# protolambda/go-kzg

Measured on AMD Instinct MI355X. Metric: KZG commitments/sec (CommitToPoly, 4096-element blob); FK20 half: value_fk20_4096, higher is better.
Workload: dtype u32; 1 GPU; CommitToPoly, 4096-coeff blobs, eth/trusted_setup.json monomial setup (s=1337), 4096 blobs/step/GPU resident in HBM, fixed-base table budget 110 GB (library default 110 GB: signed 16-bit windows, 8 of them walked by both GLV halves of every scalar, 103 GB; see table_sweep); global_batch=4096, parallelism=dp1 (independent blobs, no data-path collective)

## Files before the change

go-kzg_amd/__init__.py:

```python
import ctypes as C
import os

import numpy as np

_HERE = os.path.dirname(os.path.abspath(__file__))
LIB_PATH = os.environ.get("KZG_HIP_LIB") or os.path.join(_HERE, "libkzg_hip.so")

OK, ERR_TOO_WIDE, ERR_NOT_POW2, ERR_LEN_MISMATCH, ERR_UPPER_HALF, ERR_BAD_ARG, ERR_BAD_POINT, ERR_NO_DEVICE, ERR_HIP, ERR_UNSUPPORTED, ERR_RECOVERY, ERR_BAD_BLOB = range(12)


class KzgError(Exception):

    def __init__(self, status, msg=""):
        super().__init__("kzg_hip status %d %s" % (status, msg))
        self.status = status


class KzgPanic(KzgError):
    """The reference panics (kzg.go:22-27,44-52,74-91; fk20_single.go:60-62,140-154; bls_kilic.go:133-135)."""


class NoDeviceError(KzgError):
    pass

# ... 47 lines not shown
        "kzg_hip_check_proof_multi_interpolation": (i32, [vp, vp, u64, vp, vp, vp]),
        "kzg_hip_toeplitz_part2": (i32, [vp, vp, vp, u64, vp]), "kzg_hip_toeplitz_part3": (i32, [vp, vp, u64, vp]),
        "kzg_hip_fk20_single_settings_new": (i32, [vp, u64, pp]), "kzg_hip_fk20_single_settings_free": (None, [vp]),
        "kzg_hip_fk20_single_x_ext_fft": (i32, [vp, vp]), "kzg_hip_fk20_single": (i32, [vp, vp, u64, vp]),
        "kzg_hip_fk20_single_batch": (i32, [vp, vp, u64, u64, vp]), "kzg_hip_fk20_single_batch_dev": (i32, [vp, vp, u64, u64, vp, vp]),
        "kzg_hip_fk20_single_da_optimized": (i32, [vp, vp, u64, vp]), "kzg_hip_da_using_fk20": (i32, [vp, vp, u64, vp]),
        "kzg_hip_da_using_fk20_batch": (i32, [vp, vp, u64, u64, vp]), "kzg_hip_da_using_fk20_batch_dev": (i32, [vp, vp, u64, u64, vp, vp]),
        "kzg_hip_fk20_multi_settings_new": (i32, [vp, u64, u64, pp]), "kzg_hip_fk20_multi_settings_free": (None, [vp]),
        "kzg_hip_fk20_multi": (i32, [vp, vp, u64, vp]), "kzg_hip_fk20_multi_da_optimized": (i32, [vp, vp, u64, vp]),
        "kzg_hip_da_using_fk20_multi": (i32, [vp, vp, u64, vp]),
        "kzg_hip_da_using_fk20_multi_batch_dev": (i32, [vp, vp, u64, u64, vp, vp]),
        "kzg_hip_fk20_multi_hext_slice_dev": (i32, [vp, vp, u64, u64, u64, vp, vp]),
        "kzg_hip_fk20_multi_finish_dev": (i32, [vp, vp, i32, vp, vp]),
        "kzg_hip_eth_settings_new": (i32, [vp, vp, u64, pp]), "kzg_hip_eth_settings_free": (None, [vp]),
        "kzg_hip_eth_blob_to_kzg_commitment_batch": (i32, [vp, vp, u64, vp, vp]),
        "kzg_hip_eth_compute_kzg_proof": (i32, [vp, vp, u64, vp, vp, vp]),
        "kzg_hip_eth_compute_kzg_proof_batch": (i32, [vp, vp, u64, u64, vp, vp, vp, vp]),
        "kzg_hip_eth_compute_kzg_proof_batch_dev": (i32, [vp, vp, u64, u64, vp, vp, vp, vp, vp]),
        "kzg_hip_eth_compute_aggregate_kzg_proof": (i32, [vp, vp, u64, vp, vp]),
        "kzg_hip_eth_compute_aggregated_poly_and_commitment": (i32, [vp, vp, vp, u64, vp, vp, vp, vp]),
        "kzg_hip_test_sha256": (None, [vp, u64, vp]),
        "kzg_hip_evaluate_poly_in_evaluation_form": (i32, [vp, vp, u64, vp, u32, vp]),
        "kzg_hip_eth_evaluate_polynomial_in_evaluation_form": (i32, [vp, vp, u64, vp, vp]),
        "kzg_hip_bench_threads_fft_fr": (i32, [vp, vp, u64, u64, u32, u32, vp, C.POINTER(C.c_double)]),
        "kzg_hip_bench_drop_in_eth_proof": (i32, [vp, vp, u64, u64, u32, u32, vp, C.POINTER(C.c_double)]),
        "kzg_hip_zero_poly_via_multiplication": (i32, [vp, vp, u64, u64, vp, vp]),
        "kzg_hip_recover_poly_from_samples": (i32, [vp, vp, vp, u64, vp]),
        "kzg_hip_calibrate": (i32, [vp, C.POINTER(C.c_double), C.POINTER(C.c_double), C.POINTER(C.c_double)]),
        "kzg_hip_bench_drop_in": (i32, [vp, i32, vp, u64, u64, u32, u32, vp, C.POINTER(C.c_double)]),
        "kzg_hip_coalesce_stats": (i32, [vp, i32, C.POINTER(u64)]),
        "kzg_hip_lincomb_promotions": (i32, [vp, C.POINTER(u64), C.POINTER(u64)]),
        "kzg_hip_test_fp_inv": (i32, [vp, vp, u64, vp, vp, C.POINTER(C.c_double), C.POINTER(C.c_double)]),
        "kzg_hip_test_fr_inv": (i32, [vp, vp, u64, vp, vp, vp]),
        "kzg_hip_kzg_table_info": (i32, [vp, C.POINTER(C.c_uint32), C.POINTER(C.c_uint32), C.POINTER(u64)]), "kzg_hip_kzg_table_additions": (u32, [vp]), "kzg_hip_kzg_set_projective_outputs": (i32, [vp, i32]),
        "kzg_hip_da_using_fk20_multi_batch": (i32, [vp, vp, u64, u64, vp]),
        "kzg_hip_multi_settings_new": (i32, [C.POINTER(i32), u32, u32, vp, u64, pp]), "kzg_hip_multi_settings_free": (None, [vp]),
        "kzg_hip_multi_device_count": (u32, [vp]), "kzg_hip_multi_device": (i32, [vp, u32]),
        "kzg_hip_multi_fft": (vp, [vp, u32]), "kzg_hip_multi_kzg": (vp, [vp, u32]),
        "kzg_hip_multi_transport": (C.c_char_p, [vp]), "kzg_hip_multi_transport_note": (C.c_char_p, [vp]), "kzg_hip_multi_transport_check": (C.c_char_p, [vp]), "kzg_hip_multi_exchanges": (u64, [vp]),
        "kzg_hip_multi_set_fft_sharding": (i32, [vp, i32]), "kzg_hip_multi_set_table_budget_gb": (i32, [vp, C.c_double]),
        "kzg_hip_multi_commit_to_poly_batch": (i32, [vp, vp, u64, u64, vp]),
        "kzg_hip_multi_compute_proof_single_batch": (i32, [vp, vp, u64, u64, vp, vp]),
        "kzg_hip_multi_fft_fr_batch": (i32, [vp, vp, u64, u64, i32, vp]), "kzg_hip_multi_das_fft_extension_batch": (i32, [vp, vp, u64, u64]),
        "kzg_hip_multi_eth_settings_new": (i32, [vp, vp, u64, pp]), "kzg_hip_multi_eth_settings_free": (None, [vp]),
        "kzg_hip_multi_eth_blob_to_kzg_commitment_batch": (i32, [vp, vp, u64, vp, vp]),
        "kzg_hip_multi_eth_compute_kzg_proof_batch": (i32, [vp, vp, u64, u64, vp, vp, vp, vp]),
        "kzg_hip_multi_fk20_single_settings_new": (i32, [vp, u64, pp]), "kzg_hip_multi_fk20_single_settings_free": (None, [vp]),
        "kzg_hip_multi_da_using_fk20_batch": (i32, [vp, vp, u64, u64, vp]), "kzg_hip_multi_da_using_fk20": (i32, [vp, vp, u64, vp]),
        "kzg_hip_multi_fk20_multi_settings_new": (i32, [vp, u64, u64, pp]), "kzg_hip_multi_fk20_multi_settings_free": (None, [vp]),
        "kzg_hip_multi_da_using_fk20_multi_batch": (i32, [vp, vp, u64, u64, vp]), "kzg_hip_multi_da_using_fk20_multi": (i32, [vp, vp, u64, vp]),
        "kzg_hip_bench_poly_lincomb_dev": (i32, [vp, vp, u64, vp, u64, u64, vp, vp]),
        "kzg_hip_prof_reset": (None, [vp, i32]), "kzg_hip_prof_read": (i32, [vp, C.c_char_p, C.POINTER(C.c_double), C.POINTER(u64)]),
    }
    for name, (res, args) in sig.items():
        if os.environ.get("KZG_HIP_LIB_ALLOW_MISSING") and not hasattr(L, name):
            continue
        f = getattr(L, name)
        f.restype, f.argtypes = res, args
    _lib = L
    return L


API_SYMBOLS = None


def device_count():
# ... 707 lines not shown
```

go-kzg_amd/csrc/capi_bench.hip:

```cpp
#include "capi_common.hpp"

namespace {
struct prof_rec { std::string name; hipEvent_t e0, e1; };
std::mutex g_prof_mu;
bool g_prof_on = false;
std::vector<prof_rec> g_prof;
}
namespace kzg {
void prof_begin(hipStream_t s, const char *name) {
    if (!g_prof_on) return;
    std::lock_guard<std::mutex> lk(g_prof_mu);
    prof_rec r; r.name = name;
    hipEventCreate(&r.e0); hipEventCreate(&r.e1);
    hipEventRecord(r.e0, s);
    g_prof.push_back(r);
}
void prof_end(hipStream_t s, const char *name) {
    if (!g_prof_on) return;
    std::lock_guard<std::mutex> lk(g_prof_mu);
    for (size_t i = g_prof.size(); i-- > 0;)
        if (g_prof[i].name == name) { hipEventRecord(g_prof[i].e1, s); break; }
}
}

// ... 150 lines not shown
    HIPCHK(hipMemcpyAsync(d_in.p, in_fp, n * sizeof(fp), hipMemcpyHostToDevice, s));
    hipEvent_t e0, e1;
    HIPCHK(hipEventCreate(&e0)); HIPCHK(hipEventCreate(&e1));
    for (int which = 0; which < 2; which++) {
        void *out = which ? out_lane : out_coop; double *ms = which ? ms_lane : ms_coop;
        if (!out) continue;
        hipEventRecord(e0, s);
        launch_fp_inv_both(s, d_in.p, d_a.p, d_b.p, n, which ? 2 : 1);
        hipEventRecord(e1, s);
        HIPCHK(hipMemcpyAsync(out, which ? d_b.p : d_a.p, n * sizeof(fp), hipMemcpyDeviceToHost, s));
        HIPCHK(hipStreamSynchronize(s));
        float t = 0; hipEventElapsedTime(&t, e0, e1);
        if (ms) *ms = t;
    }
    hipEventDestroy(e0); hipEventDestroy(e1);
    HIPCHK(hipGetLastError());
    return KZG_HIP_OK;
}
int kzg_hip_test_fr_inv(kzg_hip_fft *fs, const void *in_fr, uint64_t n, void *out_coop, void *out_lane, void *out_block) {
    if (!fs || !in_fr || !n || n > (1u << 20) || !out_coop || !out_lane || !out_block) return KZG_HIP_ERR_BAD_ARG;
    dev_guard g(fs);
    hipStream_t s = fs->stream;
    dtmp<fr> d_in(s), d_a(s), d_b(s), d_c(s);
    CHK(d_in.alloc(n)); CHK(d_a.alloc(n)); CHK(d_b.alloc(n)); CHK(d_c.alloc(n));
    HIPCHK(hipMemcpyAsync(d_in.p, in_fr, n * sizeof(fr), hipMemcpyHostToDevice, s));
    launch_fr_inv_test(s, d_in.p, n, d_a.p, d_b.p, d_c.p);
    HIPCHK(hipGetLastError());
    HIPCHK(hipMemcpyAsync(out_coop, d_a.p, n * sizeof(fr), hipMemcpyDeviceToHost, s));
    HIPCHK(hipMemcpyAsync(out_lane, d_b.p, n * sizeof(fr), hipMemcpyDeviceToHost, s));
    HIPCHK(hipMemcpyAsync(out_block, d_c.p, n * sizeof(fr), hipMemcpyDeviceToHost, s));
    HIPCHK(hipStreamSynchronize(s));
    return KZG_HIP_OK;
}
int kzg_hip_coalesce_stats(kzg_hip_kzg *ks, int op, uint64_t out[8]) {
    if (!ks || !out || op < 0 || op > 1) return KZG_HIP_ERR_BAD_ARG;
    for (int i = 0; i < 8; i++) out[i] = 0;
    std::lock_guard<std::mutex> lk(ks->fs->mu);
    coalescer *co = op == 0 ? ks->co_commit.get() : ks->co_proof.get();
    if (co) co->stats(out);
    return KZG_HIP_OK;
}
void kzg_hip_prof_reset(kzg_hip_fft *fs, int enable) {
    (void)fs;
    std::lock_guard<std::mutex> lk(g_prof_mu);
    for (auto &r : g_prof) { hipEventDestroy(r.e0); hipEventDestroy(r.e1); }
    g_prof.clear();
    g_prof_on = enable != 0;
}
int kzg_hip_prof_read(kzg_hip_fft *fs, const char *kernel, double *total_ms, uint64_t *launches) {
    if (!fs || !kernel) return KZG_HIP_ERR_BAD_ARG;
    std::lock_guard<std::mutex> lk(g_prof_mu);
    double tot = 0; uint64_t cnt = 0;
    for (auto &r : g_prof) {
        if (r.name != kernel) continue;
        HIPCHK(hipEventSynchronize(r.e1));
        float ms = 0;
        HIPCHK(hipEventElapsedTime(&ms, r.e0, r.e1));
        tot += ms; cnt++;
    }
    if (total_ms) *total_ms = tot;
    if (launches) *launches = cnt;
    return KZG_HIP_OK;
}
```

go-kzg_amd/csrc/capi_kzg.hip:

```cpp
#include "capi_common.hpp"

int kzg_settings_build(kzg_hip_fft *fs, const void *points_g1, uint64_t n, kzg_hip_kzg **out) {
    dev_guard g(fs);
    hipStream_t s = fs->stream;
    std::unique_ptr<kzg_hip_kzg, void (*)(kzg_hip_kzg *)> own(new kzg_hip_kzg, kzg_hip_kzg_settings_free);
    kzg_hip_kzg *ks = own.get();
    ks->fs = fs; ks->n_setup = n;
    dtmp<g1j> d_raw(s);
    CHK(d_raw.alloc(n));
    HIPCHK(hipMalloc((void **)&ks->d_secret, n * sizeof(g1j)));
    HIPCHK(hipMalloc((void **)&ks->d_secret_a, n * sizeof(g1a)));
    HIPCHK(hipMemcpyAsync(d_raw.p, points_g1, n * sizeof(g1j), hipMemcpyHostToDevice, s));
    launch_g1_from_kilic(s, d_raw.p, n);
    launch_g1_normalize(s, d_raw.p, ks->d_secret, n);
    launch_g1_to_affine(s, ks->d_secret, ks->d_secret_a, n);
    HIPCHK(hipGetLastError());
    HIPCHK(hipStreamSynchronize(s));
    *out = own.release();
    return KZG_HIP_OK;
}
int kzg_hip_kzg_settings_new(kzg_hip_fft *fs, const void *secret_g1, uint64_t n_setup, kzg_hip_kzg **out) {
    if (!fs || !out || !secret_g1) return KZG_HIP_ERR_BAD_ARG;
    *out = nullptr;
    if (n_setup < fs->W) return KZG_HIP_ERR_LEN_MISMATCH;
// ... 35 lines not shown
}
int ensure_fixed_table(kzg_hip_kzg *ks, hipStream_t) {
    if (ks->d_fixed || ks->fixed_plan.c == 0xffffffffu) return KZG_HIP_OK;
    hipStream_t s = ks->fs->stream;
    double budget_gb = ks->budget_gb >= 0.0 ? ks->budget_gb : table_budget_gb("KZG_HIP_FB_BUDGET_GB", FB_DEFAULT_BUDGET_GB, 24.0);
    if (ks->n_setup < 64) { ks->fixed_plan.c = 0xffffffffu; return KZG_HIP_OK; }
    const bool glv = fb_glv_enabled();
    for (uint32_t c = 16; c >= 5; c--) {
        if (glv ? (c == 14) : (c == 15)) continue;
        const uint32_t nwin = glv ? fb_windows_glv(c) : fb_windows(c);
        double bytes = (double)nwin * (double)ks->n_setup * (double)(1u << (c - 1)) * sizeof(g1a);
        if (bytes > budget_gb * 1e9) continue;
        msm_plan p{};
        p.c = c; p.nwin = nwin; p.nb = 1u << (c - 1); p.ngroups = 1; p.fixed = 1; p.glv = glv ? 1 : 0; p.table_n = ks->n_setup;
        size_t entries = (size_t)p.nwin * ks->n_setup * p.nb;
        g1a *tab = nullptr;
        if (hipMalloc((void **)&tab, entries * sizeof(g1a)) != hipSuccess) { (void)hipGetLastError(); continue; }
        hipError_t e = launch_fb_build(s, ks->d_secret_a, ks->n_setup, p.c, p.nwin, tab);
        if (e == hipSuccess) e = hipStreamSynchronize(s);
        if (e != hipSuccess) { (void)hipGetLastError(); hipFree(tab); continue; }
        ks->d_fixed = tab; ks->fixed_plan = p;
        return KZG_HIP_OK;
    }
    ks->fixed_plan.c = 0xffffffffu;
    return KZG_HIP_OK;
}

int commit_rows(kzg_hip_kzg *ks, hipStream_t s, const fr *d_sc, uint64_t n, uint64_t batch, g1j *d_out, uint64_t sc_stride, bool to_kilic) {
    CHK(ensure_fixed_table(ks, s));
    bool fixed = ks->d_fixed != nullptr;
    if (!sc_stride) sc_stride = n;
    msm_plan p = fixed ? ks->fixed_plan : classic_plan(ks->n_setup);
    if (!fixed && !msm_index_range_ok(p, n)) return KZG_HIP_ERR_TOO_WIDE;
    size_t ws_main = fixed ? fb_partials_bytes(n, batch) : msm_workspace_bytes(p, n, batch);
    dtmp<uint8_t> d_ws(s);
    CHK(d_ws.alloc(ws_main));
    if (fixed) launch_fb_msm(s, ks->d_fixed, p.table_n, p.c, p.nwin, d_sc, sc_stride, n, batch, d_ws.p, d_out, to_kilic, p.glv != 0, to_kilic && ks->projective.load(std::memory_order_relaxed));
    else launch_msm(s, p, ks->d_secret_a, d_sc, sc_stride, n, batch, d_ws.p, d_out, to_kilic);
    HIPCHK(hipGetLastError());
    return KZG_HIP_OK;
}
int kzg_hip_kzg_set_table_budget_gb(kzg_hip_kzg *ks, double gb) {
    if (!ks || !(gb >= 0.0)) return KZG_HIP_ERR_BAD_ARG;
    std::unique_lock<std::shared_mutex> tl(ks->tab_mu);
    dev_guard g(ks->fs);
    if (ks->d_fixed) { HIPCHK(hipDeviceSynchronize()); HIPCHK(hipFree(ks->d_fixed)); ks->d_fixed = nullptr; }
    ks->fixed_plan = msm_plan{};
    ks->budget_gb = gb;
    return KZG_HIP_OK;
}

int kzg_hip_commit_to_poly_batch_dev(kzg_hip_kzg *ks, const void *d_coeffs_fr, uint64_t n, uint64_t batch, void *d_out_g1, void *stream) {
    if (!ks || !d_out_g1) return KZG_HIP_ERR_BAD_ARG;
    if (n > ks->n_setup) return KZG_HIP_ERR_LEN_MISMATCH;
    if (!batch) return KZG_HIP_OK;
    if (n == 0 || !d_coeffs_fr) return KZG_HIP_ERR_BAD_ARG;
    dev_guard g(ks->fs);
    return commit_rows(ks, (hipStream_t)stream, (const fr *)d_coeffs_fr, n, batch, (g1j *)d_out_g1);
}
namespace {
std::mutex g_reg_mu;
std::map<uintptr_t, size_t> g_registered;
}
const void *host_mapped_pointer(const void *host, size_t bytes) {
    hipPointerAttribute_t a;
    if (hipPointerGetAttributes(&a, host) != hipSuccess) { (void)hipGetLastError(); return nullptr; }
    if (a.type != hipMemoryTypeHost || !a.devicePointer) return nullptr;
// ... 359 lines not shown
```

go-kzg_amd/csrc/internal.hpp:

```cpp
#pragma once
#include <hip/hip_runtime.h>
#include <stdint.h>
#include "field.hpp"
#include "g1.hpp"

namespace kzg {

void launch_fr_fft(hipStream_t s, const fr *in, uint64_t in_stride, uint64_t n_in, fr *out, uint64_t n, uint64_t batch,
                   const fr *roots, uint64_t W, const fr *scale, const uint32_t *tw4096 = nullptr, const fr *roots_l = nullptr);
void launch_das_ext(hipStream_t s, fr *vals, uint64_t n, uint64_t batch, const fr *expanded, const fr *reversed, uint64_t W,
                    const fr *inv_n, const uint32_t *tw2048 = nullptr);
void launch_toeplitz_coeffs(hipStream_t s, const fr *poly, uint64_t poly_stride, uint64_t n, uint64_t l, uint64_t batch, fr *out,
                            const fr *scale);
void launch_quotient_linear(hipStream_t s, const fr *poly, uint64_t poly_stride, uint64_t n, uint64_t batch, const fr *x, fr *q, uint64_t q_stride);
void launch_fr_from_u64(hipStream_t s, const uint64_t *in, uint64_t in_stride, fr *out, uint64_t n);
void launch_fr_zero_tails(hipStream_t s, fr *rows, uint64_t n_max, uint64_t batch, const uint64_t *lens, uint64_t lens_stride);
void launch_fr_any_nonzero(hipStream_t s, const fr *vals, uint64_t n, uint32_t *flag);
void launch_fr_powers(hipStream_t s, const fr *base, uint64_t n, fr *out);

void launch_fr_from_le32(hipStream_t s, const uint8_t *in, fr *out, uint64_t per_blob, uint64_t batch, uint32_t *bad);
void launch_fr_to_le32(hipStream_t s, const fr *in, uint8_t *out, uint64_t n);
void launch_fr_bitrev_gather(hipStream_t s, const fr *in, fr *out, uint64_t n);
constexpr uint64_t ZERO_TREE_LEAF = 16;
void launch_zero_leaves(hipStream_t s, const fr *expanded, uint64_t stride, const uint64_t *missing, uint64_t n_missing, uint64_t leaves, fr *a);
// ... 26 lines not shown
void launch_g1_stage_coop_dif(hipStream_t s, int lanes, g1j *data, uint64_t n, uint64_t batch, uint64_t m, const fr *roots, const int8_t *wnaf, uint64_t W, uint64_t total);
void launch_g1_stage_coop_dit(hipStream_t s, int lanes, g1j *data, uint64_t n, uint64_t batch, uint64_t m, const fr *roots, const int8_t *wnaf, uint64_t W, uint64_t total);
void launch_g1_direct_coop(hipStream_t s, int lanes, uint32_t wgs, size_t pad_lds, const g1j *src, uint64_t src_stride, uint64_t src_valid, g1j *dst, uint32_t logn, uint32_t logR,
                           uint64_t Ns, const fr *roots, uint64_t W, const fr *sc, uint64_t total, uint32_t logT, uint32_t logU);
void launch_g1_fft_direct(hipStream_t s, const g1j *in, uint64_t in_stride, uint64_t n_valid, g1j *data, g1j *tmp, uint64_t n, uint64_t batch, const fr *roots,
                          uint64_t W, const fr *scale, uint32_t max_logr = 4, int lanes = 1, uint32_t bits_done = 0, uint64_t n_out = 0);
void launch_g1_normalize(hipStream_t s, const g1j *in, g1j *out, uint64_t n, bool to_kilic = false);
void launch_fr_inv_test(hipStream_t s, const fr *in, uint64_t n, fr *out_coop, fr *out_lane, fr *out_block);
void launch_fp_inv_both(hipStream_t s, const fp *in, fp *out_coop, fp *out_lane, uint64_t n, int mode);
void launch_g1_from_kilic(hipStream_t s, g1j *data, uint64_t n);
void launch_g1_to_affine(hipStream_t s, const g1j *in, g1a *out, uint64_t n);
void launch_g1_compress(hipStream_t s, const g1j *in, uint8_t *out48, uint64_t n);
void launch_g1_decompress(hipStream_t s, const uint8_t *in48, g1j *out, uint64_t n, uint32_t *bad_flag);
void launch_g1_fixed_base_powers(hipStream_t s, const fr *powers, uint64_t n, g1j *out);

uint64_t device_simd_lanes();
inline uint64_t device_simds() { return device_simd_lanes() / 64; }
struct msm_plan {
    uint32_t c;
    uint32_t nwin;
    uint32_t nb;
    uint32_t ngroups;
    uint32_t fixed;
    uint32_t glv;
    uint64_t table_n;
};
inline bool msm_index_range_ok(const msm_plan &p, uint64_t n) { return n < (1ull << 27) && 2 * p.table_n < (1ull << 30); }
size_t msm_workspace_bytes(const msm_plan &p, uint64_t n, uint64_t batch);
void launch_msm(hipStream_t s, const msm_plan &p, const g1a *table, const fr *scalars, uint64_t sc_stride, uint64_t n, uint64_t batch, void *workspace, g1j *out,
                bool to_kilic);
void launch_msm_window_table(hipStream_t s, const g1a *pts, uint64_t n, uint32_t c, uint32_t nwin, g1j *tmp, g1a *out);

size_t fb_partials_bytes(uint64_t n, uint64_t batch);
hipError_t launch_fb_build(hipStream_t s, const g1a *pts, uint64_t n, uint32_t c, uint32_t nwin, g1a *table);
void launch_fb_msm(hipStream_t s, const g1a *table, uint64_t table_n, uint32_t c, uint32_t nwin, const fr *scalars, uint64_t sc_stride, uint64_t n,
                   uint64_t batch, void *partials, g1j *out, bool to_kilic, bool glv = false, bool projective = false);

void launch_fb_mul_vec(hipStream_t s, const g1a *table, uint64_t table_n, uint32_t c, uint32_t nwin, const fr *scalars, uint64_t row, uint64_t j0,
                       uint64_t cnt, uint64_t batch, g1j *out, bool glv = false);
void launch_fb_mul_vec_dif2(hipStream_t s, const g1a *table, uint64_t table_n, uint32_t c, uint32_t nwin, const fr *scalars, const fr *roots, uint64_t W,
                            uint64_t batch, g1j *out, bool glv = false);
void launch_fb_mul_vec_files(hipStream_t s, const g1a *table, uint64_t table_n, uint32_t c, uint32_t nwin, const fr *scalars, uint64_t row, uint64_t j0,
                             uint64_t cnt, uint64_t batch, g1j *out, bool glv = false);
void launch_g1_sum_files(hipStream_t s, const g1j *tmp, uint64_t nfiles, uint64_t cnt, uint64_t batch, g1j *out);

void prof_begin(hipStream_t s, const char *name);
void prof_end(hipStream_t s, const char *name);

}
```

go-kzg_amd/csrc/k_msm.hip:

```cpp
#include "internal.hpp"
#include "g1_quad.hpp"
#include "coop_inv.hpp"
#include <atomic>
#include <cstring>

namespace kzg {

#define MSM_SORT_T 1024
#define MSM_ACC_BLOCK 128
#define MSM_NB 128

struct fb_partial { uint32_t w[52]; uint32_t inf; };
__device__ __forceinline__ void fb_partial_store(fb_partial &o, const g1x_acc &a) {
#pragma unroll
    for (int i = 0; i < 13; i++) { o.w[i] = a.v.x.l[i]; o.w[13 + i] = a.v.y.l[i]; o.w[26 + i] = a.v.zz.l[i]; o.w[39 + i] = a.v.zzz.l[i]; }
    o.inf = a.inf ? 1u : 0u;
}
__device__ __forceinline__ void fb_partial_load(const fb_partial &p, g1xq &v) {
#pragma unroll
    for (int i = 0; i < 13; i++) { v.x.l[i] = p.w[i]; v.y.l[i] = p.w[13 + i]; v.zz.l[i] = p.w[26 + i]; v.zzz.l[i] = p.w[39 + i]; }
}

template <uint32_t DELTA, bool ROW> __device__ __forceinline__ uint32_t lane_down(uint32_t v) {
    if constexpr (ROW && DELTA < 16) return (uint32_t)__builtin_amdgcn_update_dpp((int)v, (int)v, 0x100 + DELTA, 0xf, 0xf, false);
// ... 459 lines not shown
    hipLaunchKernelGGL(k_msm_sort, dim3((uint32_t)batch), dim3(MSM_SORT_T), sh, s, p.ngroups, p.table_n, scalars, sc_stride, n, ws, L.per_blob, L.entries_off,
                       L.offsets_off, K2);
    uint32_t S = 1;
    while (S < 16 && batch * L.K * S * 2 <= 2 * device_simd_lanes()) S *= 2;
    uint64_t total = batch * L.K * S;
    static const int seg_mode = [] { const char *e = getenv("KZG_HIP_MSM_SEG"); return e ? atoi(e) : -1; }();
    prof_begin(s, "msm_accumulate");
    const bool balanced = seg_mode == 1 || (seg_mode < 0 && batch * L.nseg >= 2 * device_simd_lanes());
    if (balanced) {
        const uint64_t tseg = batch * L.nseg, tb = batch * L.K;
        hipLaunchKernelGGL(k_msm_accumulate_seg, dim3((uint32_t)((tseg + MSM_ACC_BLOCK - 1) / MSM_ACC_BLOCK)), dim3(MSM_ACC_BLOCK), 0, s, table, ws, L.per_blob,
                           L.entries_off, L.offsets_off, L.buckets_off, L.segs_off, K2, L.nseg, tseg);
        hipLaunchKernelGGL(k_msm_merge_segs, dim3((uint32_t)((tb + MSM_ACC_BLOCK - 1) / MSM_ACC_BLOCK)), dim3(MSM_ACC_BLOCK), 0, s, ws, L.per_blob, L.offsets_off,
                           L.buckets_off, L.segs_off, K, tb);
    } else
        hipLaunchKernelGGL(k_msm_accumulate, dim3((uint32_t)((total + MSM_ACC_BLOCK - 1) / MSM_ACC_BLOCK)), dim3(MSM_ACC_BLOCK), 0, s, table, ws, L.per_blob,
                           L.entries_off, L.offsets_off, L.buckets_off, K, S, total);
    prof_end(s, "msm_accumulate");
    static const int reduce_mode = [] { const char *e = getenv("KZG_HIP_MSM_REDUCE"); return !e ? -1 : !strcmp(e, "chunks") ? 1 : !strcmp(e, "scan") ? 0 : -1; }();
    if (reduce_mode == 1 || (reduce_mode < 0 && balanced && batch * p.ngroups * 32 >= device_simd_lanes())) {
        const uint64_t tg = batch * p.ngroups;
        hipLaunchKernelGGL(k_msm_reduce_chunks, dim3((uint32_t)((tg + 3) / 4)), dim3(MSM_NB), 0, s, ws, L.per_blob, L.buckets_off, L.gsum_off, p.ngroups, tg);
    } else
        hipLaunchKernelGGL(k_msm_reduce, dim3((uint32_t)(batch * p.ngroups)), dim3(MSM_NB), 0, s, ws, L.per_blob, L.buckets_off, L.gsum_off, p.ngroups);
    hipLaunchKernelGGL(k_msm_combine, dim3((uint32_t)((batch + 63) / 64)), dim3(256), 0, s, ws, L.per_blob, L.gsum_off, p.ngroups, batch, out, to_kilic ? 1 : 0);
}

#ifndef FB_BLOCK
#define FB_BLOCK 128
#endif
#ifndef FB_FINISH_LANES_MAX
#define FB_FINISH_LANES_MAX 4
#endif
#ifndef FB_KEEP
#define FB_KEEP 16
#endif
#ifndef FB_ACC_WAVES
#define FB_ACC_WAVES 2
#endif

__global__ __launch_bounds__(FB_BLOCK, 2) void k_fb_build_pass1(const g1a *rows, uint64_t lanes, uint32_t D, uint32_t S, g1a *table, fp *ztmp) {
    uint64_t t = blockIdx.x * (uint64_t)blockDim.x + threadIdx.x;
    const uint32_t segs = D / S;
    if (t >= lanes * segs) return;
    const uint64_t row = t / segs; const uint32_t seg = (uint32_t)(t % segs);
    g1a b = rows[row];
    g1j cur = to_jac(b);
    uint32_t k = seg * S + 1;
    if (k > 1) {
        cur = g1_inf();
#pragma nounroll
        for (int bit = 31 - __builtin_clz(k); bit >= 0; bit--) {
            cur = g1_dbl(cur);
            if ((k >> bit) & 1u) cur = g1_madd(cur, b);
        }
    }
    g1a *dst = table + row * D + (uint64_t)seg * S; fp *zd = ztmp + row * D + (uint64_t)seg * S;
#pragma nounroll
    for (uint32_t d = 0; d < S; d++) {
        g1a xy; xy.x = cur.x; xy.y = cur.y;
        dst[d] = xy; zd[d] = cur.z;
        cur = g1_madd(cur, b);
    }
}
__global__ __launch_bounds__(FB_BLOCK, 2) void k_fb_build_pass2(uint64_t lanes, uint32_t D, uint32_t S, g1a *table, fp *ztmp, fp *ptmp) {
    uint64_t t = blockIdx.x * (uint64_t)blockDim.x + threadIdx.x;
    if (t >= lanes * (D / S)) return;
    g1a *dst = table + t * S; fp *zd = ztmp + t * S; fp *pd = ptmp + t * S;
    fp acc = one<FpP>();
// ... 143 lines not shown
            if (cmag) {
#else
        g1a qn = table[((uint64_t)w0 * table_n + i) * D + (mag ? mag - 1 : 0)];
#pragma nounroll
        for (uint32_t w = w0; w < w1; w++) {
            g1a q = qn;
            const uint32_t cmag = mag, cng = ng;
            if (w + 1 < w1) {
                raw = scalar_bits(k, (w + 1) * c, c) + carry;
                if (raw > D) { carry = 1; mag = (1u << c) - raw; ng = 1; } else { carry = 0; mag = raw; ng = 0; }
                qn = table[((uint64_t)(w + 1) * table_n + i) * D + (mag ? mag - 1 : 0)];
            }
            if (cmag) {
#endif
                if (cng) q.y = neg<FpP>(q.y);
                acc.add(q);
            }
        }
    }
#ifdef KZG_REDUCE_WAVE_COOP
    fb_block_reduce_coop(acc, buf, &lds, tid);
#else
    fb_block_reduce_quad(acc, buf, tid);
#endif
    if (tid == 0) fb_partial_store(partials[blockIdx.x], acc);
}
__device__ __forceinline__ uint32_t mag_bits(const uint32_t (&m)[4], uint32_t off, uint32_t c) {
    const uint32_t idx = off >> 5, sh = off & 31;
    if (idx >= 4) return 0;
    uint64_t v = m[idx];
    if (idx + 1 < 4) v |= (uint64_t)m[idx + 1] << 32;
    return (uint32_t)(v >> sh) & ((1u << c) - 1u);
}
template <bool SPLIT> __global__ __launch_bounds__(FB_ACC_BLOCK, FB_ACC_WAVES) void k_fb_accumulate_glv(const g1a *table, uint64_t table_n, uint32_t c, uint32_t nwin, uint32_t D, const fr *scalars,
                                                            uint64_t sc_stride, uint64_t n, uint32_t blocks_per_blob, uint32_t wsplit, fb_partial *partials) {
    __shared__ fb_partial buf[64];
#ifdef KZG_REDUCE_WAVE_COOP
    __shared__ coop_lds lds;
#endif
    const uint32_t tid = threadIdx.x;
    const uint64_t blob = blockIdx.x / blocks_per_blob; const uint32_t blk = blockIdx.x % blocks_per_blob;
    const uint64_t L = (uint64_t)blocks_per_blob * FB_ACC_BLOCK;
    const fr *sc = scalars + blob * sc_stride;
    g1x_acc acc; acc.init();
    const uint32_t wpg = SPLIT ? (nwin + wsplit - 1) / wsplit : nwin;
    const uint64_t nvh = SPLIT ? n * wsplit : n;
    bool in_phi = false;
    const bool keep_ok = !SPLIT && nvh % L == 0 && nvh / L <= FB_KEEP;
    uint32_t kept[FB_KEEP][5];
    uint32_t slot = 0;
    for (uint64_t v = (uint64_t)blk * FB_ACC_BLOCK + tid; v < 2 * nvh; v += L) {
        const bool phi = v < nvh;
        const uint64_t vh = phi ? v : v - nvh;
        const uint64_t i = SPLIT ? vh % n : vh;
        const uint32_t w0 = SPLIT ? (uint32_t)(vh / n) * wpg : 0u;
        const uint32_t w1 = SPLIT ? (w0 + wpg < nwin ? w0 + wpg : nwin) : nwin;
        if (SPLIT && w0 >= w1) continue;
        if (in_phi && !phi) { if (!acc.inf) acc.v.x = mulq(acc.v.x, unpackq(glv_beta())); in_phi = false; }
        uint32_t m[4], sgn;
        if (keep_ok && !phi) {
            const uint32_t at = slot < FB_KEEP ? slot : 0; slot++;
#pragma unroll
            for (int j = 0; j < 4; j++) m[j] = kept[at][j];
            sgn = kept[at][4];
            if (slot == (uint32_t)(nvh / L)) slot = 0;
        } else {
            const glv_halves h = glv_split_signed(from_mont<FrP>(sc[i]));
#pragma unroll
            for (int j = 0; j < 4; j++) m[j] = phi ? h.k2[j] : h.k1[j];
            sgn = phi ? h.neg2 : h.neg1;
            if (keep_ok) {
                const uint32_t at = slot < FB_KEEP ? slot : 0; slot++;
#pragma unroll
                for (int j = 0; j < 4; j++) kept[at][j] = h.k1[j];
                kept[at][4] = h.neg1;
                if (slot == (uint32_t)(nvh / L)) slot = 0;
            }
        }
        uint32_t raw, carry = 0, mag, ng;
        if (SPLIT) {
#pragma nounroll
            for (uint32_t w = 0; w < w0; w++) carry = (mag_bits(m, w * c, c) + carry > D) ? 1u : 0u;
        }
        raw = mag_bits(m, w0 * c, c) + carry;
        if (raw > D) { carry = 1; mag = (1u << c) - raw; ng = 1; } else { carry = 0; mag = raw; ng = 0; }
        g1a qn = table[((uint64_t)w0 * table_n + i) * D + (mag ? mag - 1 : 0)];
#pragma nounroll
        for (uint32_t w = w0; w < w1; w++) {
            g1a q = qn;
            const uint32_t cmag = mag, cng = ng;
            if (w + 1 < w1) {
                raw = mag_bits(m, (w + 1) * c, c) + carry;
                if (raw > D) { carry = 1; mag = (1u << c) - raw; ng = 1; } else { carry = 0; mag = raw; ng = 0; }
                qn = table[((uint64_t)(w + 1) * table_n + i) * D + (mag ? mag - 1 : 0)];
            }
            if (cmag) {
                if (cng ^ sgn) q.y = neg<FpP>(q.y);
                acc.add(q);
                in_phi = phi;
            }
        }
    }
    if (in_phi && !acc.inf) acc.v.x = mulq(acc.v.x, unpackq(glv_beta()));
#ifdef KZG_REDUCE_WAVE_COOP
    fb_block_reduce_coop(acc, buf, &lds, tid);
#else
    fb_block_reduce_quad(acc, buf, tid);
#endif
    if (tid == 0) fb_partial_store(partials[blockIdx.x], acc);
}
__global__ __launch_bounds__(256) void k_fb_finish(const fb_partial *partials, uint32_t blocks_per_blob, uint64_t batch, g1j *out, int to_kilic) {
    __shared__ fb_partial buf[64];
    const uint64_t b = blockIdx.x;
#ifdef KZG_REDUCE_WAVE_COOP
    __shared__ coop_lds lds;
    coop_ctx c; c.L = &lds; c.wave = threadIdx.x >> 6; c.col = threadIdx.x & 63u; c.set = 0;
    const uint32_t col = c.col;
    g1x_acc acc; acc.init();
    acc.v = g1xq_from_affine(g1a_inf());
    const uint32_t rounds = (blocks_per_blob + 63) / 64;
#pragma nounroll
    for (uint32_t r = 0; r < rounds; r++) {
        const uint32_t j = r * 64 + col;
        const bool have = j < blocks_per_blob;
        const fb_partial &pj = partials[b * blocks_per_blob + (have ? j : 0)];
        g1xq w; fb_partial_load(pj, w);
        coop_acc_add(acc, w, !have || pj.inf != 0, c);
    }
    const uint32_t live = blocks_per_blob < 64 ? blocks_per_blob : 64;
    uint32_t off = 1;
// ... 282 lines not shown
                            j0, cnt, row, total, out);
    prof_end(s, "fb_mul_vec");
}

uint64_t device_simd_lanes() {
    static std::atomic<uint64_t> lanes_of_device[64];
    int dev = 0;
    (void)hipGetDevice(&dev);
    std::atomic<uint64_t> &slot = lanes_of_device[dev >= 0 && dev < 64 ? dev : 0];
    uint64_t lanes = slot.load(std::memory_order_relaxed);
    if (!lanes) {
        int cus = 256;
        if (hipDeviceGetAttribute(&cus, hipDeviceAttributeMultiprocessorCount, dev) != hipSuccess) { (void)hipGetLastError(); cus = 256; }
        lanes = (uint64_t)(cus > 0 ? cus : 256) * 4 * 64;
        slot.store(lanes, std::memory_order_relaxed);
    }
    return lanes;
}
static uint32_t fb_blocks_per_blob(uint64_t n, uint64_t batch, uint32_t *wsplit = nullptr) {
    static const uint64_t forced_lanes = [] { const char *e = getenv("KZG_HIP_FB_LANES"); return e ? strtoull(e, nullptr, 10) : 0ull; }();
    uint64_t lanes = forced_lanes ? forced_lanes : 2 * device_simd_lanes();
    if (lanes < FB_ACC_BLOCK) lanes = FB_ACC_BLOCK;
    uint64_t target = lanes / FB_ACC_BLOCK;
    uint64_t bpb = target / (batch ? batch : 1);
    uint32_t split = 1;
    while (split < 8 && (batch ? batch : 1) * n * split * 2 <= lanes) split *= 2;
    if (wsplit) *wsplit = split;
    uint64_t maxb = (n * split + FB_ACC_BLOCK - 1) / FB_ACC_BLOCK;
    if (bpb > maxb) bpb = maxb;
    if (bpb < 1) bpb = 1;
    return (uint32_t)bpb;
}
size_t fb_partials_bytes(uint64_t n, uint64_t batch) { return (((size_t)std::max(fb_blocks_per_blob(n, batch), fb_blocks_per_blob(2 * n, batch)) * batch * sizeof(fb_partial)) + 15) / 16 * 16; }

void launch_fb_msm(hipStream_t s, const g1a *table, uint64_t table_n, uint32_t c, uint32_t nwin, const fr *scalars, uint64_t sc_stride, uint64_t n,
                   uint64_t batch, void *partials, g1j *out, bool to_kilic, bool glv, bool projective) {
    if (!batch) return;
    const int fin = (to_kilic ? 1 : 0) | (projective ? 2 : 0);
    uint32_t split = 1;
    uint32_t bpb = fb_blocks_per_blob(glv ? 2 * n : n, batch, &split);
    if (split > nwin) split = nwin;
    prof_begin(s, "fb_accumulate");
    if (glv) {
        if (split > 1) hipLaunchKernelGGL(k_fb_accumulate_glv<true>, dim3((uint32_t)(batch * bpb)), dim3(FB_ACC_BLOCK), 0, s, table, table_n, c, nwin, 1u << (c - 1), scalars, sc_stride, n,
                                          bpb, split, (fb_partial *)partials);
        else hipLaunchKernelGGL(k_fb_accumulate_glv<false>, dim3((uint32_t)(batch * bpb)), dim3(FB_ACC_BLOCK), 0, s, table, table_n, c, nwin, 1u << (c - 1), scalars, sc_stride, n, bpb,
                                1u, (fb_partial *)partials);
    } else if (split > 1) hipLaunchKernelGGL(k_fb_accumulate<true>, dim3((uint32_t)(batch * bpb)), dim3(FB_ACC_BLOCK), 0, s, table, table_n, c, nwin, 1u << (c - 1), scalars, sc_stride, n,
                                      bpb, split, (fb_partial *)partials);
    else hipLaunchKernelGGL(k_fb_accumulate<false>, dim3((uint32_t)(batch * bpb)), dim3(FB_ACC_BLOCK), 0, s, table, table_n, c, nwin, 1u << (c - 1), scalars, sc_stride, n, bpb,
                            1u, (fb_partial *)partials);
    prof_end(s, "fb_accumulate");
    if (bpb <= FB_FINISH_LANES_MAX) hipLaunchKernelGGL(k_fb_finish_lanes, dim3((uint32_t)((batch + 63) / 64)), dim3(64), 0, s, (const fb_partial *)partials, bpb, batch, out, fin);
    else hipLaunchKernelGGL(k_fb_finish, dim3((uint32_t)batch), dim3(256), 0, s, (const fb_partial *)partials, bpb, batch, out, fin);
}
hipError_t launch_fb_build(hipStream_t s, const g1a *pts, uint64_t n, uint32_t c, uint32_t nwin, g1a *table) {
    uint32_t D = 1u << (c - 1);
    g1j *rows_j = nullptr; g1a *rows = nullptr; fp *ztmp = nullptr, *ptmp = nullptr;
    uint64_t lanes_all = (uint64_t)nwin * n;
    hipError_t e;
    if ((e = hipMallocAsync((void **)&rows_j, lanes_all * sizeof(g1j), s)) != hipSuccess) return e;
    if ((e = hipMallocAsync((void **)&rows, lanes_all * sizeof(g1a), s)) != hipSuccess) { hipFreeAsync(rows_j, s); return e; }
    launch_msm_window_table(s, pts, n, c, nwin, rows_j, rows);
    uint64_t per_win = n * D * sizeof(fp);
    uint32_t slab = (uint32_t)((1ull << 30) / (per_win ? per_win : 1));
    if (slab < 1) slab = 1;
    if (slab > nwin) slab = nwin;
    if ((e = hipMallocAsync((void **)&ztmp, (uint64_t)slab * per_win, s)) != hipSuccess) { hipFreeAsync(rows_j, s); hipFreeAsync(rows, s); return e; }
    if ((e = hipMallocAsync((void **)&ptmp, (uint64_t)slab * per_win, s)) != hipSuccess) { hipFreeAsync(rows_j, s); hipFreeAsync(rows, s); hipFreeAsync(ztmp, s); return e; }
    for (uint32_t w0 = 0; w0 < nwin; w0 += slab) {
        uint32_t ws = (w0 + slab <= nwin) ? slab : nwin - w0;
        uint64_t lanes = (uint64_t)ws * n;
        uint32_t S = D;
        while (S > 64 && lanes * (D / S) < (1ull << 20)) S >>= 1;
        dim3 g((uint32_t)((lanes * (D / S) + FB_BLOCK - 1) / FB_BLOCK)), b(FB_BLOCK);
        hipLaunchKernelGGL(k_fb_build_pass1, g, b, 0, s, rows + (uint64_t)w0 * n, lanes, D, S, table + (uint64_t)w0 * n * D, ztmp);
        hipLaunchKernelGGL(k_fb_build_pass2, g, b, 0, s, lanes, D, S, table + (uint64_t)w0 * n * D, ztmp, ptmp);
    }
    hipFreeAsync(rows_j, s); hipFreeAsync(rows, s); hipFreeAsync(ztmp, s); hipFreeAsync(ptmp, s);
    return hipGetLastError();
}

__global__ __launch_bounds__(MSM_ACC_BLOCK, 2) void k_msm_window_rows(const g1a *pts, uint64_t n, uint32_t c, uint32_t nwin, g1j *tmp) {
    uint64_t i = blockIdx.x * (uint64_t)blockDim.x + threadIdx.x;
    if (i >= n) return;
// ... 16 lines not shown
```

go-kzg_amd/csrc/kzg_hip_internal.h:

```cpp
#ifndef KZG_HIP_INTERNAL_H
#define KZG_HIP_INTERNAL_H
#include "../../include/kzg_hip.h"
#ifdef __cplusplus
extern "C" {
#endif
#pragma GCC visibility push(default)

void kzg_hip_prof_reset(kzg_hip_fft *fs, int enable);
int kzg_hip_prof_read(kzg_hip_fft *fs, const char *kernel, double *total_ms, uint64_t *launches);
int kzg_hip_calibrate(kzg_hip_fft *fs, double *mad_per_s, double *add_per_s, double *fp_mul_per_s);
int kzg_hip_bench_drop_in(kzg_hip_kzg *ks, int op, const void *blobs_fr, uint64_t n, uint64_t nblobs, unsigned threads, unsigned calls, void *out_g1,
                          double *seconds);
int kzg_hip_bench_drop_in_eth_proof(kzg_hip_eth *eth, const void *polys_fr, uint64_t n, uint64_t npolys, unsigned threads, unsigned calls, void *out48,
                                    double *seconds);
int kzg_hip_bench_threads_fft_fr(kzg_hip_fft *fs, const void *vals_fr, uint64_t n, uint64_t nrows, unsigned threads, unsigned calls, void *out_fr, double *seconds);
int kzg_hip_bench_poly_lincomb_dev(kzg_hip_fft *fs, const void *d_vectors_fr, uint64_t stride, const void *d_scalars_fr, uint64_t count, uint64_t n, void *d_out_fr,
                                   void *stream);
int kzg_hip_coalesce_stats(kzg_hip_kzg *ks, int op, uint64_t out[8]);
int kzg_hip_test_fp_inv(kzg_hip_fft *fs, const void *in_fp, uint64_t n, void *out_coop, void *out_lane, double *ms_coop, double *ms_lane);
int kzg_hip_lincomb_promotions(kzg_hip_fft *fs, uint64_t *promoted, uint64_t *served);
int kzg_hip_test_fr_inv(kzg_hip_fft *fs, const void *in_fr, uint64_t n, void *out_coop, void *out_lane, void *out_block);
void kzg_hip_test_sha256(const void *data, uint64_t len, void *out32);


#pragma GCC visibility pop
#ifdef __cplusplus
}
#endif
#endif
```

Baseline: 102,000 commitments/s.

## Precompute signed GLV window digits in a separate kernel before fixed-base accumulation

Adds a k_fb_digits kernel that does the GLV split and signed-window recoding once per scalar and writes int16 digits to a workspace buffer. The accumulate kernel then reads those digits instead of redoing the split and carry chain in every thread, and the FB_KEEP register cache of kept halves is removed. This is meant to take scalar decomposition and recoding arithmetic out of the accumulate hot loop and cut register pressure there. The cost is an extra kernel launch, extra HBM traffic for the digit buffer (processed in chunks capped at 1 GB), and more workspace.

Result: no change. 102,500 commitments/s (median of 6 runs) (+0.5%).

```diff
diff --git a/go-kzg_amd/__init__.py b/go-kzg_amd/__init__.py
--- a/go-kzg_amd/__init__.py
+++ b/go-kzg_amd/__init__.py
@@ -103,6 +103,7 @@
         "kzg_hip_lincomb_promotions": (i32, [vp, C.POINTER(u64), C.POINTER(u64)]),
         "kzg_hip_test_fp_inv": (i32, [vp, vp, u64, vp, vp, C.POINTER(C.c_double), C.POINTER(C.c_double)]),
         "kzg_hip_test_fr_inv": (i32, [vp, vp, u64, vp, vp, vp]),
+        "kzg_hip_test_fb_digits": (i32, [vp, vp, u64, u32, vp]),
         "kzg_hip_kzg_table_info": (i32, [vp, C.POINTER(C.c_uint32), C.POINTER(C.c_uint32), C.POINTER(u64)]), "kzg_hip_kzg_table_additions": (u32, [vp]), "kzg_hip_kzg_set_projective_outputs": (i32, [vp, i32]),
         "kzg_hip_da_using_fk20_multi_batch": (i32, [vp, vp, u64, u64, vp]),
         "kzg_hip_multi_settings_new": (i32, [C.POINTER(i32), u32, u32, vp, u64, pp]), "kzg_hip_multi_settings_free": (None, [vp]),
diff --git a/go-kzg_amd/csrc/capi_bench.hip b/go-kzg_amd/csrc/capi_bench.hip
--- a/go-kzg_amd/csrc/capi_bench.hip
+++ b/go-kzg_amd/csrc/capi_bench.hip
@@ -206,6 +206,20 @@
     HIPCHK(hipStreamSynchronize(s));
     return KZG_HIP_OK;
 }
+int kzg_hip_test_fb_digits(kzg_hip_fft *fs, const void *scalars_fr, uint64_t n, uint32_t c, void *out_i16) {
+    if (!fs || !scalars_fr || !n || n > (1u << 20) || c < 2 || c > 16 || !out_i16) return KZG_HIP_ERR_BAD_ARG;
+    dev_guard g(fs);
+    hipStream_t s = fs->stream;
+    const uint32_t nwin = fb_windows_glv(c);
+    dtmp<fr> d_in(s); dtmp<int16_t> d_out(s);
+    CHK(d_in.alloc(n)); CHK(d_out.alloc(2ull * nwin * n));
+    HIPCHK(hipMemcpyAsync(d_in.p, scalars_fr, n * sizeof(fr), hipMemcpyHostToDevice, s));
+    launch_fb_digits(s, d_in.p, n, n, 1, c, nwin, d_out.p);
+    HIPCHK(hipGetLastError());
+    HIPCHK(hipMemcpyAsync(out_i16, d_out.p, 2ull * nwin * n * sizeof(int16_t), hipMemcpyDeviceToHost, s));
+    HIPCHK(hipStreamSynchronize(s));
+    return KZG_HIP_OK;
+}
 int kzg_hip_coalesce_stats(kzg_hip_kzg *ks, int op, uint64_t out[8]) {
     if (!ks || !out || op < 0 || op > 1) return KZG_HIP_ERR_BAD_ARG;
     for (int i = 0; i < 8; i++) out[i] = 0;
diff --git a/go-kzg_amd/csrc/capi_kzg.hip b/go-kzg_amd/csrc/capi_kzg.hip
--- a/go-kzg_amd/csrc/capi_kzg.hip
+++ b/go-kzg_amd/csrc/capi_kzg.hip
@@ -91,7 +91,7 @@
     if (!sc_stride) sc_stride = n;
     msm_plan p = fixed ? ks->fixed_plan : classic_plan(ks->n_setup);
     if (!fixed && !msm_index_range_ok(p, n)) return KZG_HIP_ERR_TOO_WIDE;
-    size_t ws_main = fixed ? fb_partials_bytes(n, batch) : msm_workspace_bytes(p, n, batch);
+    size_t ws_main = fixed ? fb_msm_workspace_bytes(n, batch, p.nwin, p.glv != 0) : msm_workspace_bytes(p, n, batch);
     dtmp<uint8_t> d_ws(s);
     CHK(d_ws.alloc(ws_main));
     if (fixed) launch_fb_msm(s, ks->d_fixed, p.table_n, p.c, p.nwin, d_sc, sc_stride, n, batch, d_ws.p, d_out, to_kilic, p.glv != 0, to_kilic && ks->projective.load(std::memory_order_relaxed));
diff --git a/go-kzg_amd/csrc/internal.hpp b/go-kzg_amd/csrc/internal.hpp
--- a/go-kzg_amd/csrc/internal.hpp
+++ b/go-kzg_amd/csrc/internal.hpp
@@ -82,9 +82,11 @@
 void launch_msm_window_table(hipStream_t s, const g1a *pts, uint64_t n, uint32_t c, uint32_t nwin, g1j *tmp, g1a *out);
 
 size_t fb_partials_bytes(uint64_t n, uint64_t batch);
+size_t fb_msm_workspace_bytes(uint64_t n, uint64_t batch, uint32_t nwin, bool glv);
+void launch_fb_digits(hipStream_t s, const fr *scalars, uint64_t sc_stride, uint64_t n, uint64_t batch, uint32_t c, uint32_t nwin, int16_t *digits);
 hipError_t launch_fb_build(hipStream_t s, const g1a *pts, uint64_t n, uint32_t c, uint32_t nwin, g1a *table);
 void launch_fb_msm(hipStream_t s, const g1a *table, uint64_t table_n, uint32_t c, uint32_t nwin, const fr *scalars, uint64_t sc_stride, uint64_t n,
-                   uint64_t batch, void *partials, g1j *out, bool to_kilic, bool glv = false, bool projective = false);
+                   uint64_t batch, void *workspace, g1j *out, bool to_kilic, bool glv = false, bool projective = false);
 
 void launch_fb_mul_vec(hipStream_t s, const g1a *table, uint64_t table_n, uint32_t c, uint32_t nwin, const fr *scalars, uint64_t row, uint64_t j0,
                        uint64_t cnt, uint64_t batch, g1j *out, bool glv = false);
diff --git a/go-kzg_amd/csrc/k_msm.hip b/go-kzg_amd/csrc/k_msm.hip
--- a/go-kzg_amd/csrc/k_msm.hip
+++ b/go-kzg_amd/csrc/k_msm.hip
@@ -515,9 +515,6 @@
 #ifndef FB_FINISH_LANES_MAX
 #define FB_FINISH_LANES_MAX 4
 #endif
-#ifndef FB_KEEP
-#define FB_KEEP 16
-#endif
 #ifndef FB_ACC_WAVES
 #define FB_ACC_WAVES 2
 #endif
@@ -727,8 +724,28 @@
     if (idx + 1 < 4) v |= (uint64_t)m[idx + 1] << 32;
     return (uint32_t)(v >> sh) & ((1u << c) - 1u);
 }
-template <bool SPLIT> __global__ __launch_bounds__(FB_ACC_BLOCK, FB_ACC_WAVES) void k_fb_accumulate_glv(const g1a *table, uint64_t table_n, uint32_t c, uint32_t nwin, uint32_t D, const fr *scalars,
-                                                            uint64_t sc_stride, uint64_t n, uint32_t blocks_per_blob, uint32_t wsplit, fb_partial *partials) {
+__device__ __forceinline__ void fb_recode_half(const uint32_t (&m)[4], uint32_t neg, uint32_t c, uint32_t nwin, int16_t *dst, uint64_t stride) {
+    const uint32_t D = 1u << (c - 1);
+    uint32_t carry = 0;
+#pragma nounroll
+    for (uint32_t w = 0; w < nwin; w++) {
+        const uint32_t raw = mag_bits(m, w * c, c) + carry;
+        carry = neg ? (raw > D ? 1u : 0u) : (raw >= D ? 1u : 0u);
+        const int32_t d = (int32_t)raw - (int32_t)(carry << c);
+        dst[(uint64_t)w * stride] = (int16_t)(neg ? -d : d);
+    }
+}
+__global__ __launch_bounds__(256) void k_fb_digits(const fr *scalars, uint64_t sc_stride, uint64_t n, uint64_t batch, uint32_t c, uint32_t nwin, int16_t *digits) {
+    const uint64_t t = (uint64_t)blockIdx.x * 256 + threadIdx.x;
+    if (t >= n * batch) return;
+    const uint64_t b = t / n, i = t - b * n;
+    const glv_halves h = glv_split_signed(from_mont<FrP>(scalars[b * sc_stride + i]));
+    int16_t *dst = digits + b * 2 * nwin * n + i;
+    fb_recode_half(h.k2, h.neg2, c, nwin, dst, n);
+    fb_recode_half(h.k1, h.neg1, c, nwin, dst + (uint64_t)nwin * n, n);
+}
+template <bool SPLIT> __global__ __launch_bounds__(FB_ACC_BLOCK, FB_ACC_WAVES) void k_fb_accumulate_glv(const g1a *table, uint64_t table_n, uint32_t nwin, uint32_t D, const int16_t *digits,
+                                                            uint64_t n, uint32_t blocks_per_blob, uint32_t wsplit, fb_partial *partials) {
     __shared__ fb_partial buf[64];
 #ifdef KZG_REDUCE_WAVE_COOP
     __shared__ coop_lds lds;
@@ -736,14 +753,11 @@
     const uint32_t tid = threadIdx.x;
     const uint64_t blob = blockIdx.x / blocks_per_blob; const uint32_t blk = blockIdx.x % blocks_per_blob;
     const uint64_t L = (uint64_t)blocks_per_blob * FB_ACC_BLOCK;
-    const fr *sc = scalars + blob * sc_stride;
+    const int16_t *dg = digits + blob * 2 * nwin * n;
     g1x_acc acc; acc.init();
     const uint32_t wpg = SPLIT ? (nwin + wsplit - 1) / wsplit : nwin;
     const uint64_t nvh = SPLIT ? n * wsplit : n;
     bool in_phi = false;
-    const bool keep_ok = !SPLIT && nvh % L == 0 && nvh / L <= FB_KEEP;
-    uint32_t kept[FB_KEEP][5];
-    uint32_t slot = 0;
     for (uint64_t v = (uint64_t)blk * FB_ACC_BLOCK + tid; v < 2 * nvh; v += L) {
         const bool phi = v < nvh;
         const uint64_t vh = phi ? v : v - nvh;
@@ -752,45 +766,19 @@
         const uint32_t w1 = SPLIT ? (w0 + wpg < nwin ? w0 + wpg : nwin) : nwin;
         if (SPLIT && w0 >= w1) continue;
         if (in_phi && !phi) { if (!acc.inf) acc.v.x = mulq(acc.v.x, unpackq(glv_beta())); in_phi = false; }
-        uint32_t m[4], sgn;
-        if (keep_ok && !phi) {
-            const uint32_t at = slot < FB_KEEP ? slot : 0; slot++;
-#pragma unroll
-            for (int j = 0; j < 4; j++) m[j] = kept[at][j];
-            sgn = kept[at][4];
-            if (slot == (uint32_t)(nvh / L)) slot = 0;
-        } else {
-            const glv_halves h = glv_split_signed(from_mont<FrP>(sc[i]));
-#pragma unroll
-            for (int j = 0; j < 4; j++) m[j] = phi ? h.k2[j] : h.k1[j];
-            sgn = phi ? h.neg2 : h.neg1;
-            if (keep_ok) {
-                const uint32_t at = slot < FB_KEEP ? slot : 0; slot++;
-#pragma unroll
-                for (int j = 0; j < 4; j++) kept[at][j] = h.k1[j];
-                kept[at][4] = h.neg1;
-                if (slot == (uint32_t)(nvh / L)) slot = 0;
-            }
-        }
-        uint32_t raw, carry = 0, mag, ng;
-        if (SPLIT) {
-#pragma nounroll
-            for (uint32_t w = 0; w < w0; w++) carry = (mag_bits(m, w * c, c) + carry > D) ? 1u : 0u;
-        }
-        raw = mag_bits(m, w0 * c, c) + carry;
-        if (raw > D) { carry = 1; mag = (1u << c) - raw; ng = 1; } else { carry = 0; mag = raw; ng = 0; }
-        g1a qn = table[((uint64_t)w0 * table_n + i) * D + (mag ? mag - 1 : 0)];
+        const uint32_t off = (phi ? 0u : nwin) * (uint32_t)n + (uint32_t)i, nn = (uint32_t)n;
+        int32_t e = dg[off + w0 * nn];
+        int32_t en = dg[off + (w0 + 1 < w1 ? w0 + 1 : w0) * nn];
+        g1a qn = table[((uint64_t)w0 * table_n + i) * D + (e ? (uint32_t)abs(e) - 1 : 0u)];
 #pragma nounroll
         for (uint32_t w = w0; w < w1; w++) {
             g1a q = qn;
-            const uint32_t cmag = mag, cng = ng;
-            if (w + 1 < w1) {
-                raw = mag_bits(m, (w + 1) * c, c) + carry;
-                if (raw > D) { carry = 1; mag = (1u << c) - raw; ng = 1; } else { carry = 0; mag = raw; ng = 0; }
-                qn = table[((uint64_t)(w + 1) * table_n + i) * D + (mag ? mag - 1 : 0)];
-            }
-            if (cmag) {
-                if (cng ^ sgn) q.y = neg<FpP>(q.y);
+            const int32_t ce = e;
+            e = en;
+            en = dg[off + (w + 2 < w1 ? w + 2 : w1 - 1) * nn];
+            if (w + 1 < w1) qn = table[((uint64_t)(w + 1) * table_n + i) * D + (e ? (uint32_t)abs(e) - 1 : 0u)];
+            if (ce) {
+                if (ce < 0) q.y = neg<FpP>(q.y);
                 acc.add(q);
                 in_phi = phi;
             }
@@ -1139,25 +1127,54 @@
     return (uint32_t)bpb;
 }
 size_t fb_partials_bytes(uint64_t n, uint64_t batch) { return (((size_t)std::max(fb_blocks_per_blob(n, batch), fb_blocks_per_blob(2 * n, batch)) * batch * sizeof(fb_partial)) + 15) / 16 * 16; }
+#ifndef FB_DIGITS_MAX_BYTES
+#define FB_DIGITS_MAX_BYTES (1ull << 30)
+#endif
+static uint64_t fb_digits_chunk(uint64_t n, uint32_t nwin, uint64_t batch) {
+    const uint64_t per_blob = 2ull * nwin * n * sizeof(int16_t);
+    const uint64_t cb = FB_DIGITS_MAX_BYTES / per_blob;
+    return std::max<uint64_t>(1, std::min<uint64_t>(batch, cb));
+}
+size_t fb_msm_workspace_bytes(uint64_t n, uint64_t batch, uint32_t nwin, bool glv) {
+    const size_t parts = fb_partials_bytes(n, batch);
+    return glv ? parts + fb_digits_chunk(n, nwin, batch) * 2ull * nwin * n * sizeof(int16_t) : parts;
+}
+void launch_fb_digits(hipStream_t s, const fr *scalars, uint64_t sc_stride, uint64_t n, uint64_t batch, uint32_t c, uint32_t nwin, int16_t *digits) {
+    const uint64_t t = n * batch;
+    hipLaunchKernelGGL(k_fb_digits, dim3((uint32_t)((t + 255) / 256)), dim3(256), 0, s, scalars, sc_stride, n, batch, c, nwin, digits);
+}
 
 void launch_fb_msm(hipStream_t s, const g1a *table, uint64_t table_n, uint32_t c, uint32_t nwin, const fr *scalars, uint64_t sc_stride, uint64_t n,
-                   uint64_t batch, void *partials, g1j *out, bool to_kilic, bool glv, bool projective) {
+                   uint64_t batch, void *workspace, g1j *out, bool to_kilic, bool glv, bool projective) {
     if (!batch) return;
     const int fin = (to_kilic ? 1 : 0) | (projective ? 2 : 0);
+    fb_partial *partials = (fb_partial *)workspace;
     uint32_t split = 1;
     uint32_t bpb = fb_blocks_per_blob(glv ? 2 * n : n, batch, &split);
     if (split > nwin) split = nwin;
-    prof_begin(s, "fb_accumulate");
     if (glv) {
-        if (split > 1) hipLaunchKernelGGL(k_fb_accumulate_glv<true>, dim3((uint32_t)(batch * bpb)), dim3(FB_ACC_BLOCK), 0, s, table, table_n, c, nwin, 1u << (c - 1), scalars, sc_stride, n,
-                                          bpb, split, (fb_partial *)partials);
-        else hipLaunchKernelGGL(k_fb_accumulate_glv<false>, dim3((uint32_t)(batch * bpb)), dim3(FB_ACC_BLOCK), 0, s, table, table_n, c, nwin, 1u << (c - 1), scalars, sc_stride, n, bpb,
-                                1u, (fb_partial *)partials);
-    } else if (split > 1) hipLaunchKernelGGL(k_fb_accumulate<true>, dim3((uint32_t)(batch * bpb)), dim3(FB_ACC_BLOCK), 0, s, table, table_n, c, nwin, 1u << (c - 1), scalars, sc_stride, n,
-                                      bpb, split, (fb_partial *)partials);
-    else hipLaunchKernelGGL(k_fb_accumulate<false>, dim3((uint32_t)(batch * bpb)), dim3(FB_ACC_BLOCK), 0, s, table, table_n, c, nwin, 1u << (c - 1), scalars, sc_stride, n, bpb,
-                            1u, (fb_partial *)partials);
-    prof_end(s, "fb_accumulate");
+        int16_t *digits = (int16_t *)((uint8_t *)workspace + fb_partials_bytes(n, batch));
+        const uint64_t chunk = fb_digits_chunk(n, nwin, batch);
+        for (uint64_t b0 = 0; b0 < batch; b0 += chunk) {
+            const uint64_t cb = std::min(chunk, batch - b0);
+            prof_begin(s, "fb_digits");
+            launch_fb_digits(s, scalars + b0 * sc_stride, sc_stride, n, cb, c, nwin, digits);
+            prof_end(s, "fb_digits");
+            prof_begin(s, "fb_accumulate");
+            if (split > 1) hipLaunchKernelGGL(k_fb_accumulate_glv<true>, dim3((uint32_t)(cb * bpb)), dim3(FB_ACC_BLOCK), 0, s, table, table_n, nwin, 1u << (c - 1), digits, n,
+                                              bpb, split, partials + b0 * bpb);
+            else hipLaunchKernelGGL(k_fb_accumulate_glv<false>, dim3((uint32_t)(cb * bpb)), dim3(FB_ACC_BLOCK), 0, s, table, table_n, nwin, 1u << (c - 1), digits, n, bpb,
+                                    1u, partials + b0 * bpb);
+            prof_end(s, "fb_accumulate");
+        }
+    } else {
+        prof_begin(s, "fb_accumulate");
+        if (split > 1) hipLaunchKernelGGL(k_fb_accumulate<true>, dim3((uint32_t)(batch * bpb)), dim3(FB_ACC_BLOCK), 0, s, table, table_n, c, nwin, 1u << (c - 1), scalars, sc_stride, n,
+                                          bpb, split, partials);
+        else hipLaunchKernelGGL(k_fb_accumulate<false>, dim3((uint32_t)(batch * bpb)), dim3(FB_ACC_BLOCK), 0, s, table, table_n, c, nwin, 1u << (c - 1), scalars, sc_stride, n, bpb,
+                                1u, partials);
+        prof_end(s, "fb_accumulate");
+    }
     if (bpb <= FB_FINISH_LANES_MAX) hipLaunchKernelGGL(k_fb_finish_lanes, dim3((uint32_t)((batch + 63) / 64)), dim3(64), 0, s, (const fb_partial *)partials, bpb, batch, out, fin);
     else hipLaunchKernelGGL(k_fb_finish, dim3((uint32_t)batch), dim3(256), 0, s, (const fb_partial *)partials, bpb, batch, out, fin);
 }
diff --git a/go-kzg_amd/csrc/kzg_hip_internal.h b/go-kzg_amd/csrc/kzg_hip_internal.h
--- a/go-kzg_amd/csrc/kzg_hip_internal.h
+++ b/go-kzg_amd/csrc/kzg_hip_internal.h
@@ -20,6 +20,7 @@
 int kzg_hip_test_fp_inv(kzg_hip_fft *fs, const void *in_fp, uint64_t n, void *out_coop, void *out_lane, double *ms_coop, double *ms_lane);
 int kzg_hip_lincomb_promotions(kzg_hip_fft *fs, uint64_t *promoted, uint64_t *served);
 int kzg_hip_test_fr_inv(kzg_hip_fft *fs, const void *in_fr, uint64_t n, void *out_coop, void *out_lane, void *out_block);
+int kzg_hip_test_fb_digits(kzg_hip_fft *fs, const void *scalars_fr, uint64_t n, uint32_t c, void *out_i16);
 void kzg_hip_test_sha256(const void *data, uint64_t len, void *out32);
 
 
```
